# zhengchen1999/DOVE

Hardware: AMD Instinct MI355X
Metric: SR frames/s (33x720x1280 4x one-step, whole job) (higher is better)
Workload: dtype bf16; 1 GPU; synthetic 33x720x1280 HR clip (LR 180x320, 4x), one-step t=399, CogVideoX1.5-5B VAE + 42-layer DiT random-init, 1 clip per GPU (BASELINE configs[1]); weight_sums=True, vae_streams=2, variant=headline (bf16)

## Files before the change

### dove_amd/csrc/igemm.hip

```cpp
#include "igemm_args.h"


template <int BN, int BK>
struct FastCfg {
  static constexpr int BM = 128;
  static constexpr int CPR = BK / 8;
  static constexpr int CPR_LOG = (BK == 64) ? 3 : 2;
  static constexpr int RPG = 256 / CPR;
  static constexpr int NA = BM / RPG;
  static constexpr int B_SLOTS = BN * CPR;
  static constexpr int NB = (B_SLOTS + 255) / 256;
  static constexpr int A_BYTES = BM * BK * 2, B_BYTES = BN * BK * 2, STAGE = A_BYTES + B_BYTES;
  static constexpr int WN = (BN >= 128) ? 2 : 1, WM = 4 / WN;
  static constexpr int PT = (BM / WM) / 32, CT = (BN / WN) / 32;
  static constexpr int KK = BK / 16;
};

template <int BN, int BK>
__global__ __launch_bounds__(256) void igemm_fast_kernel(const IgemmArgs a) {
  using Cf = FastCfg<BN, BK>;
  constexpr int NA = Cf::NA, NB = Cf::NB, PT = Cf::PT, CT = Cf::CT, KK = Cf::KK, STAGE = Cf::STAGE, A_BYTES = Cf::A_BYTES;
  extern __shared__ __attribute__((aligned(16))) char smem[];
  const int tid = threadIdx.x, lane = tid & 63;
  const int wave = __builtin_amdgcn_readfirstlane(tid >> 6);
  __builtin_assume(wave >= 0 && wave < 4);
  const int wm = wave / Cf::WN, wn = wave % Cf::WN;

  unsigned rest = xcd_remap(blockIdx.x, gridDim.x);
  const int tn = rest % a.tiles_n; rest /= a.tiles_n;
  const int twi = rest % a.tiles_w; rest /= a.tiles_w;
  const int thi = rest % a.tiles_h;
  const int t = rest / a.tiles_h;
  const int n0 = tn * BN;
  const int TWm = (1 << a.tw_log2) - 1;
  const int oh0 = thi * (128 >> a.tw_log2), ow0 = twi << a.tw_log2;

  const int cs = tid & (Cf::CPR - 1);
  const int rsub = tid >> Cf::CPR_LOG;
  const int c = (BK == 64) ? (cs ^ ((rsub >> 1) & 7)) : (cs ^ ((rsub >> 2) & 3));
  int rowoff[NA];
  unsigned mask[NA];
#pragma unroll
  for (int j = 0; j < NA; ++j) {
    const int m = j * Cf::RPG + rsub;
    const int oh = oh0 + (m >> a.tw_log2), ow = ow0 + (m & TWm);
    const bool mv = (oh < a.H_out) && (ow < a.W_out);
    const int ih0 = oh * a.stride - a.pad_h, iw0 = ow * a.stride - a.pad_w;
    rowoff[j] = ((ih0 * a.W_in + iw0) * a.Cin + c * 8) * 2;
    unsigned mk = 0;
    for (int dh = 0; dh < a.kh; ++dh)
      for (int dw = 0; dw < a.kw; ++dw) {
        const bool ok = mv && ((unsigned)(ih0 + dh) < (unsigned)a.H_in) && ((unsigned)(iw0 + dw) < (unsigned)a.W_in);
        mk |= (ok ? 1u : 0u) << (dh * a.kw + dw);
      }
    mask[j] = mk;
  }
  int boff_g[NB];
#pragma unroll
  for (int j = 0; j < NB; ++j) boff_g[j] = ((j * Cf::RPG + rsub) * a.Cin + c * 8) * 2;

  const long long frame_elems = (long long)a.H_in * a.W_in * a.Cin;
  const unsigned frame_bytes = (unsigned)(frame_elems * 2);
  const unsigned wtap_bytes = (unsigned)((long long)BN * a.Cin * 2);
  const long long wtap_stride = (long long)a.Cout_pad * a.Cin;
  const int kc_per_tap = a.Cin / BK;
  const int nk = a.kt * a.kh * a.kw * kc_per_tap;

  auto frame_ptr = [&](int dt) -> const bf16_t* { return igemm_src_frame(a, t, dt, frame_elems); };
  int s_kc = 0, s_dw = 0, s_dh = 0, s_dt = 0;
  const bf16_t* s_fp = frame_ptr(0);
  const bf16_t* s_wp = a.w + (long long)n0 * a.Cin;
  int s_tapdelta = 0;
  unsigned s_tapbit = 1u;

// ... 23 lines not shown
          ++s_dt;
          if (s_dt < a.kt) s_fp = frame_ptr(s_dt);
        }
      }
      s_tapdelta = ((s_dh * a.W_in + s_dw) * a.Cin) * 2;
      s_tapbit = 1u << (s_dh * a.kw + s_dw);
    }
  };

  const int hi = lane >> 5, l31 = lane & 31;
  int aoff[PT][KK], boff[CT][KK];
#pragma unroll
  for (int kk = 0; kk < KK; ++kk) {
    const int chunk = kk * 2 + hi;
#pragma unroll
    for (int p = 0; p < PT; ++p) {
      const int row = wm * (Cf::BM / Cf::WM) + p * 32 + l31;
      const int sc = (BK == 64) ? (chunk ^ ((row >> 1) & 7)) : (chunk ^ ((row >> 2) & 3));
      aoff[p][kk] = row * (BK * 2) + sc * 16;
    }
#pragma unroll
    for (int i = 0; i < CT; ++i) {
      const int row = wn * (BN / Cf::WN) + i * 32 + l31;
      const int sc = (BK == 64) ? (chunk ^ ((row >> 1) & 7)) : (chunk ^ ((row >> 2) & 3));
      boff[i][kk] = row * (BK * 2) + sc * 16;
    }
  }

  f32x16 acc[CT][PT];
#pragma unroll
  for (int i = 0; i < CT; ++i)
#pragma unroll
    for (int p = 0; p < PT; ++p)
#pragma unroll
      for (int r = 0; r < 16; ++r) acc[i][p][r] = 0.f;

  auto compute = [&](auto bufc) {
    constexpr int BUF = decltype(bufc)::value;
#pragma unroll
    for (int kk = 0; kk < KK; ++kk) {
      bf16x8 xf[PT], wf[CT];
#pragma unroll
      for (int p = 0; p < PT; ++p) xf[p] = *(const bf16x8*)(smem + BUF * STAGE + aoff[p][kk]);
#pragma unroll
      for (int i = 0; i < CT; ++i) wf[i] = *(const bf16x8*)(smem + BUF * STAGE + A_BYTES + boff[i][kk]);
#pragma unroll
      for (int i = 0; i < CT; ++i)
#pragma unroll
        for (int p = 0; p < PT; ++p)
          acc[i][p] = __builtin_amdgcn_mfma_f32_32x32x16_bf16(wf[i], xf[p], acc[i][p], 0, 0, 0);
    }
  };

  using B0 = std::integral_constant<int, 0>;
  using B1 = std::integral_constant<int, 1>;
  stage(B0{});
  int it = 0;
  for (; it + 2 <= nk; it += 2) {
    asm volatile("s_waitcnt vmcnt(0)" ::: "memory");
    __syncthreads();
    stage(B1{});
    compute(B0{});
    asm volatile("s_waitcnt vmcnt(0)" ::: "memory");
    __syncthreads();
    if (it + 2 < nk) stage(B0{});
    compute(B1{});
  }
  if (nk & 1) {
    asm volatile("s_waitcnt vmcnt(0)" ::: "memory");
    __syncthreads();
    compute(B0{});
  }

#pragma unroll
  for (int p = 0; p < PT; ++p) {
    const int m = wm * (Cf::BM / Cf::WM) + p * 32 + l31;
    const int oh = oh0 + (m >> a.tw_log2), ow = ow0 + (m & TWm);
    if (!((oh < a.H_out) && (ow < a.W_out))) continue;
    const long long pix = ((long long)t * a.H_out + oh) * a.W_out + ow;
    const float* gate = a.gate ? (a.gate + (pix < a.gate_split ? 0 : a.Cout_pad)) : nullptr;
#pragma unroll
    for (int i = 0; i < CT; ++i) {
#pragma unroll
      for (int g = 0; g < 4; ++g) {
        const int cb = n0 + wn * (BN / Cf::WN) + i * 32 + 8 * g + 4 * hi;
        if (cb >= a.Cout_st) continue;
        float v[4];
#pragma unroll
        for (int e = 0; e < 4; ++e) v[e] = acc[i][p][g * 4 + e];
        if (a.bias) {
          const f32x4 b = *(const f32x4*)(a.bias + cb);
#pragma unroll
          for (int e = 0; e < 4; ++e) v[e] += b[e];
        }
        if (a.act == 1) {
#pragma unroll
          for (int e = 0; e < 4; ++e) v[e] = gelu_tanh_f(v[e]);
        }
        if (a.resid) {
          const uint2 rr = *(const uint2*)(a.resid + pix * a.ldr + cb);
          float r[4] = {__uint_as_float(rr.x << 16), __uint_as_float(rr.x & 0xffff0000u),
                        __uint_as_float(rr.y << 16), __uint_as_float(rr.y & 0xffff0000u)};
          if (gate) {
            const f32x4 gg = *(const f32x4*)(gate + cb);
#pragma unroll
            for (int e = 0; e < 4; ++e) v[e] = r[e] + gg[e] * v[e];
          } else {
#pragma unroll
            for (int e = 0; e < 4; ++e) v[e] += r[e];
          }
        }
        uint2 o;
        o.x = pack_bf2(v[0], v[1]);
        o.y = pack_bf2(v[2], v[3]);
        if (a.out_f32) *(f32x4*)((float*)a.out + pix * a.ldo + cb) = f32x4{v[0], v[1], v[2], v[3]};
        else *(uint2*)(a.out + pix * a.ldo + cb) = o;
      }
    }
  }
}


namespace halo8 {
constexpr int TH = 16, TW = 32, HWID = TW + 2, HHGT = TH + 2, HPIX = HWID * HHGT;
// ... 870 lines not shown
      for (int j = 0; j < 4; ++j)
        acc[j] = __builtin_amdgcn_fdot2_f32_bf16(__builtin_bit_cast(v2bf, wr[j][k]), __builtin_bit_cast(v2bf, xr[k]), acc[j], false);
    uint2 o;
    o.x = pack_bf2(acc[0], acc[1]);
    o.y = pack_bf2(acc[2], acc[3]);
    *(uint2*)(out + m * ldo + n0) = o;
  }
}

enum ConvKernel { K_IGEMM = 0, K_IGEMM_FAST, K_HALO4X, K_HALO4X_UP, K_GEMM8P, K_SMALLK, K_HALO4X_SUB };
static const char* const kKernelNames[] = {"igemm_kernel", "igemm_fast_kernel", "conv3x3_halo4x_kernel", "conv3x3_halo4x_kernel", "gemm8p_kernel",
                                           "smallk_kernel", "conv3x3_halo4x_kernel"};

static inline int desc_nb(const dove_conv_desc* d) { return d->nb > 1 ? d->nb : 1; }

static ConvKernel select_kernel(const dove_conv_desc* d) {
  const long long M = (long long)desc_nb(d) * d->t_out * d->h_out * d->w_out;
  const bool frame_fits = (long long)d->h_in * d->w_in * d->cin * 2 < (1ll << 31);
  const bool plain_gemm = d->kt == 1 && d->kh == 1 && d->kw == 1 && d->stride == 1 && d->up == 0 && d->tmode == 0 &&
                          d->t_in == d->t_out && d->h_in == d->h_out && d->w_in == d->w_out && d->cout_pad % 128 == 0 && M >= 4096 &&
                          (long long)512 * d->cin * 2 < (1ll << 31);
  const bool pointwise = d->kt == 1 && d->kh == 1 && d->kw == 1 && d->stride == 1 && d->up == 0 && d->tmode == 0 && d->t_in == d->t_out &&
                         d->h_in == d->h_out && d->w_in == d->w_out;
  if (pointwise && d->cin == 32 && d->act == 0 && !d->resid && !d->gate && d->cout_store >= 128) return K_SMALLK;
  if (plain_gemm) {
    if (d->cout_pad % 256 == 0 && d->cout_store % 256 == 0 && d->cin % 128 == 0 && d->cin >= 256 && (long long)256 * d->cin * 2 < (1ll << 31) &&
        d->ldo < (1 << 20) && d->ldr < (1 << 20) && (d->act == 0 || d->act == 1))
      return K_GEMM8P;
  }
  const bool conv3 = d->kh == 3 && d->kw == 3 && d->stride == 1 && d->pad_h == 1 && d->pad_w == 1 && d->act == 0 && !d->gate &&
                     d->cout_pad % 128 == 0 && frame_fits;
  if (conv3) {
    const bool same = d->up == 0 && d->tmode == 0 && d->h_out == d->h_in && d->w_out == d->w_in && d->w_out >= 16 && d->h_out >= 16;
    const bool ups = d->up == 1 && d->kt == 1 && d->h_out == 2 * d->h_in && d->w_out == 2 * d->w_in && d->h_out >= 16 && d->w_out >= 32;
    const bool h4 = d->cout_store % 128 == 0 && d->cin % 64 == 0 && d->ldo < (1 << 20) && (!d->resid || d->ldr < (1 << 20));
    if (same && h4) return K_HALO4X;
    if (ups && h4 && d->w_sub && d->h_in >= 16 && d->w_in >= 32) return K_HALO4X_SUB;
    if (ups && h4) return K_HALO4X_UP;
  }
  const int BN = (d->cout_pad % 128 == 0) ? 128 : ((d->cout_pad % 64 == 0) ? 64 : 32);
  const bool fits = frame_fits && (long long)BN * d->cin * 2 < (1ll << 31);
  return (d->up == 0 && fits) ? K_IGEMM_FAST : K_IGEMM;
}

static bool desc_size_ok(const dove_conv_desc* d, const char* who) {
  if (d && d->struct_size == sizeof(dove_conv_desc) && d->reserved == 0) return true;
  if (d) dove_set_error("%s: dove_conv_desc.struct_size is %u, this library (ABI %d) expects %zu - the caller's binding was written "
                        "against another include/dove_hip.h", who, d->struct_size, DOVE_ABI_VERSION, sizeof(dove_conv_desc));
  else dove_set_error("%s: null descriptor", who);
  return false;
}
extern "C" const char* dove_conv_kernel_name(const dove_conv_desc* d) { return desc_size_ok(d, "conv_kernel_name") ? kKernelNames[select_kernel(d)] : ""; }

template <int BN, int BK>
static int launch_igemm_fast(const IgemmArgs& a, unsigned grid, hipStream_t s) {
  constexpr int lds = 2 * (128 * BK * 2 + BN * BK * 2);
  static PerDeviceOnce attr_set;
  if (auto once_ = attr_set.guard()) (void)hipFuncSetAttribute((const void*)igemm_fast_kernel<BN, BK>, hipFuncAttributeMaxDynamicSharedMemorySize, lds);
  hipLaunchKernelGGL((igemm_fast_kernel<BN, BK>), dim3(grid), dim3(256), lds, s, a);
  DOVE_CHECK_LAUNCH("dove_conv_igemm_bf16");
  return DOVE_OK;
}

static int cu_count() {
  static std::atomic<int> cus[DOVE_MAX_DEVICES] = {};
  int dev = 0;
  (void)hipGetDevice(&dev);
  int n = (dev >= 0 && dev < DOVE_MAX_DEVICES) ? cus[dev].load(std::memory_order_relaxed) : 0;
  if (!n) {
    n = 256;
    (void)hipDeviceGetAttribute(&n, hipDeviceAttributeMultiprocessorCount, dev);
    if (dev >= 0 && dev < DOVE_MAX_DEVICES) cus[dev].store(n, std::memory_order_relaxed);
  }
  return n;
}

extern "C" long long dove_conv_gn_partial_rows(const dove_conv_desc* d) {
  if (!desc_size_ok(d, "conv_gn_partial_rows")) return 0;
  const ConvKernel k = select_kernel(d);
  if (k != K_HALO4X && k != K_HALO4X_UP && k != K_HALO4X_SUB) return 0;
  if (d->cout_store != 128 && d->cout_store != 256 && d->cout_store != 512) return 0;
  if (d->cout_store != d->cout_pad) return 0;
  if (k == K_HALO4X_SUB) {
    const long long th = (d->h_in + halo8::TH - 1) / halo8::TH, tw = (d->w_in + halo8::TW - 1) / halo8::TW;
    return (long long)desc_nb(d) * d->t_out * th * tw * 16;
  }
  const long long th = (d->h_out + halo8::TH - 1) / halo8::TH, tw = (d->w_out + halo8::TW - 1) / halo8::TW;
  return (long long)desc_nb(d) * d->t_out * th * tw * 4;
}

static bool halo4x_plan(const dove_conv_desc* d) {
  const int tiles_w = (d->w_out + halo8::TW - 1) / halo8::TW, tiles_h = (d->h_out + halo8::TH - 1) / halo8::TH;
  const int wrem = d->w_out % halo8::TW;
  if (wrem < 1 || wrem > halo8::TW / 2) return false;
  const int cus = cu_count();
  const long long per = (long long)desc_nb(d) * d->t_out * (d->cout_pad / 128);
  auto rounds = [&](long long tiles) { return (tiles * per + cus - 1) / cus; };
  return rounds((long long)tiles_h * (tiles_w - 1)) + rounds((d->h_out + 31) / 32) < rounds((long long)tiles_h * tiles_w);
}
extern "C" int dove_conv_partial_launches(const dove_conv_desc* d) {
  if (!desc_size_ok(d, "conv_partial_launches") || select_kernel(d) != K_HALO4X) return 0;
  return halo4x_plan(d) ? 1 : 0;
}

static int conv_dispatch(const dove_conv_desc* d, void* stream, ConvKernel kern);

static bool gemm_tail_split(const dove_conv_desc* d, long long* rows_main) {
  const long long M = (long long)d->t_out * d->h_out * d->w_out;
  if (d->t_out != 1 || d->h_out != 1 || desc_nb(d) > 1) return false;
  const int cus = cu_count(), tiles_n = d->cout_pad / 256;
  const long long row_tiles = (M + gemm4x::BM - 1) / gemm4x::BM, ntiles = row_tiles * tiles_n;
  if (ntiles <= cus || ntiles % cus == 0) return false;
  const long long main_rt = (ntiles / cus) * cus / tiles_n;
  if (main_rt < 1 || main_rt >= row_tiles) return false;
  const long long tail_rows = M - main_rt * gemm4x::BM;
  const long long tail_blocks = ((tail_rows + 127) / 128) * (d->cout_pad / 128);
  if (tail_blocks > 2ll * cus) return false;
  if ((long long)128 * d->cin * 2 >= (1ll << 31)) return false;
  *rows_main = main_rt * gemm4x::BM;
  return true;
}

extern "C" int dove_conv_igemm_bf16(const dove_conv_desc* d, void* stream) {
  if (!desc_size_ok(d, "conv_igemm")) return DOVE_EINVAL;
  DOVE_CHECK_ARG(d->x && d->w && d->out, "conv_igemm: null pointer");
  DOVE_CHECK_ARG(d->cin % 32 == 0 && d->cin > 0, "conv_igemm: Cin (%d) must be a positive multiple of 32 (pad on pack)", d->cin);
  DOVE_CHECK_ARG(d->cout_pad % 32 == 0 && d->cout_pad > 0, "conv_igemm: Cout_pad (%d) must be a multiple of 32", d->cout_pad);
  DOVE_CHECK_ARG(d->cout_store % 4 == 0 && d->cout_store <= d->cout_pad && d->cout_store > 0, "conv_igemm: bad cout_store %d", d->cout_store);
  DOVE_CHECK_ARG(d->ldo % 4 == 0 && d->ldo >= d->cout_store, "conv_igemm: ldo (%lld) must be a multiple of 4 and >= cout_store", d->ldo);
  DOVE_CHECK_ARG(!d->resid || (d->ldr % 4 == 0 && d->ldr >= d->cout_store), "conv_igemm: bad ldr %lld", d->ldr);
  DOVE_CHECK_ARG(!d->gate || d->resid, "conv_igemm: gate needs resid");
  DOVE_CHECK_ARG(d->kt >= 1 && d->kt <= 3 && d->kh >= 1 && d->kw >= 1, "conv_igemm: bad kernel size");
  DOVE_CHECK_ARG(d->stride == 1 || d->stride == 2, "conv_igemm: stride must be 1 or 2");
  DOVE_CHECK_ARG(d->up == 0 || d->up == 1, "conv_igemm: up must be 0/1");
  DOVE_CHECK_ARG(d->kt == 1 || (d->tmode == 0 && d->t_in == d->t_out), "conv_igemm: causal temporal taps need t_in == t_out and tmode 0");
  DOVE_CHECK_ARG(d->t_out > 0 && d->h_out > 0 && d->w_out > 0 && d->t_in > 0 && d->h_in > 0 && d->w_in > 0, "conv_igemm: empty tensor");
  DOVE_CHECK_ARG(d->nb >= 0 && d->nb <= 4096 && (long long)desc_nb(d) * d->t_out < (1 << 20), "conv_igemm: bad instance count nb = %d", d->nb);
  DOVE_CHECK_ARG(d->cache_stride == 0 || (d->cache && d->cache_stride >= (long long)(d->kt - 1) * d->h_in * d->w_in * d->cin),
                 "conv_igemm: cache_stride (%lld) is smaller than one instance's cache", d->cache_stride);
  DOVE_CHECK_ARG(desc_nb(d) == 1 || !d->gate, "conv_igemm: nb > 1 is not combined with gate");
  DOVE_CHECK_ARG(d->reserved2 == 0 && d->tdup >= 0 && d->tdup <= 2, "conv_igemm: bad tdup %d", d->tdup);
  DOVE_CHECK_ARG(!d->tdup || (d->kt == 3 && d->w_pair), "conv_igemm: tdup declares frame pairs of a kt == 3 conv and needs w_pair");
  DOVE_CHECK_ARG(!d->tdup || d->cache || d->w_first, "conv_igemm: tdup without a conv cache needs w_first too (frames whose three taps read one frame)");
  DOVE_CHECK_ARG(d->tdup != 2 || !d->cache, "conv_igemm: tdup == 2 (first frame single) is the head of a clip: no conv cache");
  DOVE_CHECK_ARG(!d->gn_partial || dove_conv_gn_partial_rows(d) > 0,
                 "conv_igemm: gn_partial requested but this call does not dispatch to a kernel that fuses the statistics");
  const ConvKernel kern0 = select_kernel(d);
  DOVE_CHECK_ARG(!d->out_f32 || (kern0 == K_IGEMM_FAST && !d->resid && d->act == 0),
                 "conv_igemm: out_f32 is only implemented for plain convs that dispatch to igemm_fast_kernel");
  long long rows_main = 0;
  if (kern0 == K_GEMM8P && gemm_tail_split(d, &rows_main)) {
    dove_conv_desc m = *d, t = *d;
    m.w_in = m.w_out = (int)rows_main;
    const long long tail = (long long)d->w_out - rows_main;
    t.w_in = t.w_out = (int)tail;
    t.x = (const char*)d->x + rows_main * d->cin * 2;
    t.out = (char*)d->out + rows_main * d->ldo * 2;
    if (d->resid) t.resid = (const char*)d->resid + rows_main * d->ldr * 2;
    t.gate_split = d->gate_split > rows_main ? d->gate_split - rows_main : 0;
    const int rc = conv_dispatch(&m, stream, K_GEMM8P);
    return rc ? rc : conv_dispatch(&t, stream, K_IGEMM_FAST);
  }
  return conv_dispatch(d, stream, kern0);
}

static int conv_dispatch(const dove_conv_desc* d, void* stream, ConvKernel kern) {
  const bf16_t* zp = zero_page();
  DOVE_CHECK_ARG(zp, "conv_igemm: could not allocate the zero page");
  IgemmArgs a;
  a.x = (const bf16_t*)d->x; a.cache = (const bf16_t*)d->cache; a.w = (const bf16_t*)d->w;
  a.bias = d->bias; a.resid = (const bf16_t*)d->resid; a.gate = d->gate; a.out = (bf16_t*)d->out; a.zero = zp;
  const int nb = desc_nb(d);
  a.T_out = nb * d->t_out; a.H_out = d->h_out; a.W_out = d->w_out;
  a.T_in = nb * d->t_in; a.H_in = d->h_in; a.W_in = d->w_in;
  a.seg_out = d->t_out; a.seg_in = d->t_in;
  a.cache_bs = d->cache_stride ? d->cache_stride : (long long)(d->kt - 1) * d->h_in * d->w_in * d->cin;
  a.Cin = d->cin; a.Cout_pad = d->cout_pad; a.Cout_st = d->cout_store;
  a.kt = d->kt; a.kh = d->kh; a.kw = d->kw; a.stride = d->stride; a.pad_h = d->pad_h; a.pad_w = d->pad_w;
  a.up = d->up; a.tmode = d->tmode; a.act = d->act; a.ldo = d->ldo; a.ldr = d->ldr; a.gate_split = d->gate_split;
  a.gn_partial = nullptr; a.cpg_log = 0;
  a.w_first = nullptr;
  a.w_pair = nullptr; a.tdup = 0;
  a.sub = 0;
  a.out_f32 = d->out_f32;
  a.nt_out = 0;
  a.reserved = 0;
  hipStream_t s = (hipStream_t)stream;
  const long long M = (long long)nb * d->t_out * d->h_out * d->w_out;
  switch (kern) {
    case K_GEMM8P: {
      a.tiles_n = d->cout_pad / 256;
      a.nt_out = (long long)M * d->ldo * 2 > (256ll << 20);
      const long long nt = ((M + gemm4x::BM - 1) / gemm4x::BM) * a.tiles_n;
      DOVE_CHECK_ARG(nt > 0 && nt < (1ll << 31), "conv_igemm: grid too large");
      DOVE_CHECK_ARG(!(d->gate && d->act), "conv_igemm: gate with activation is not a path of the reference");
      const int cus = cu_count();
      const unsigned grid4 = nt > cus ? (unsigned)cus : (unsigned)nt;
      static PerDeviceOnce attr8;
      if (auto once_ = attr8.guard()) {
        (void)hipFuncSetAttribute((const void*)gemm8p_kernel<false, false>, hipFuncAttributeMaxDynamicSharedMemorySize, gemm8p::LDS_BYTES);
        (void)hipFuncSetAttribute((const void*)gemm8p_kernel<true, false>, hipFuncAttributeMaxDynamicSharedMemorySize, gemm8p::LDS_BYTES);
        (void)hipFuncSetAttribute((const void*)gemm8p_kernel<false, true>, hipFuncAttributeMaxDynamicSharedMemorySize, gemm8p::LDS_BYTES);
      }
      if (d->gate) hipLaunchKernelGGL((gemm8p_kernel<false, true>), dim3(grid4), dim3(512), gemm8p::LDS_BYTES, s, a, M);
      else if (d->act == 1) hipLaunchKernelGGL((gemm8p_kernel<true, false>), dim3(grid4), dim3(512), gemm8p::LDS_BYTES, s, a, M);
      else hipLaunchKernelGGL((gemm8p_kernel<false, false>), dim3(grid4), dim3(512), gemm8p::LDS_BYTES, s, a, M);
      DOVE_CHECK_LAUNCH("dove_conv_igemm_bf16(gemm8p)");
      return DOVE_OK;
    }
    case K_SMALLK: {
      dim3 grid((unsigned)((M + 4 * smallk::ROWS - 1) / (4 * smallk::ROWS)), (unsigned)((d->cout_store + 255) / 256));
      hipLaunchKernelGGL(smallk_kernel, grid, dim3(256), 0, s, a.x, a.w, a.bias, a.out, M, d->cout_store, d->ldo);
      DOVE_CHECK_LAUNCH("dove_conv_igemm_bf16(smallk)");
      return DOVE_OK;
    }
    case K_HALO4X_SUB: {
      a.gn_partial = d->gn_partial;
      a.cpg_log = d->cout_store == 128 ? 2 : (d->cout_store == 256 ? 3 : 4);
      a.sub = 1;
// ... 4 lines not shown
      a.tiles_n = 4 * (d->cout_pad / 128);
      a.nty = a.tiles_h; a.ntx = a.tiles_w; a.h_lim = d->h_out; a.w_lim = d->w_out;
      const long long g4 = (long long)a.T_out * a.tiles_h * a.tiles_w * a.tiles_n;
      DOVE_CHECK_ARG(g4 > 0 && g4 < (1ll << 31), "conv_igemm: grid too large");
      static PerDeviceOnce attrs;
      if (auto once_ = attrs.guard()) (void)hipFuncSetAttribute((const void*)(conv3x3_halo4x_kernel<false, true>), hipFuncAttributeMaxDynamicSharedMemorySize, Halo4xCfg::LDS_BYTES);
      const int cus = cu_count();
      const unsigned grid = g4 > cus ? (unsigned)cus : (unsigned)g4;
      hipLaunchKernelGGL((conv3x3_halo4x_kernel<false, true>), dim3(grid), dim3(256), Halo4xCfg::LDS_BYTES, s, a);
      DOVE_CHECK_LAUNCH("dove_conv_igemm_bf16(halo4x sub-pixel)");
      return DOVE_OK;
    }
    case K_HALO4X:
    case K_HALO4X_UP: {
      a.gn_partial = d->gn_partial;
      a.w_first = (kern == K_HALO4X && d->kt == 3 && !d->cache) ? (const bf16_t*)d->w_first : nullptr;
      if (kern == K_HALO4X && d->kt == 3 && d->tdup) { a.tdup = d->tdup; a.w_pair = (const bf16_t*)d->w_pair; }
      a.cpg_log = d->cout_store == 128 ? 2 : (d->cout_store == 256 ? 3 : 4);
      a.tiles_w = (d->w_out + halo8::TW - 1) / halo8::TW;
      a.tiles_h = (d->h_out + halo8::TH - 1) / halo8::TH;
      a.tiles_n = d->cout_pad / 128;
      a.ty0 = a.tx0 = 0; a.nty = a.tiles_h; a.ntx = a.tiles_w; a.h_lim = d->h_out; a.w_lim = d->w_out;
      const long long g4 = (long long)a.T_out * a.tiles_h * a.tiles_w * a.tiles_n;
      DOVE_CHECK_ARG(g4 > 0 && g4 < (1ll << 31), "conv_igemm: grid too large");
      static PerDeviceOnce attr4;
      if (auto once_ = attr4.guard()) {
        (void)hipFuncSetAttribute((const void*)(conv3x3_halo4x_kernel<false>), hipFuncAttributeMaxDynamicSharedMemorySize, Halo4xCfg::LDS_BYTES);
        (void)hipFuncSetAttribute((const void*)(conv3x3_halo4x_kernel<false, false, 1>), hipFuncAttributeMaxDynamicSharedMemorySize, H4Geo<1>::LDS_BYTES);
        (void)hipFuncSetAttribute((const void*)(conv3x3_halo4x_kernel<true>), hipFuncAttributeMaxDynamicSharedMemorySize, Halo4xCfg::LDS_BYTES);
      }
      const int cus = cu_count();
      const unsigned grid = g4 > cus ? (unsigned)cus : (unsigned)g4;
      if (kern == K_HALO4X_UP) hipLaunchKernelGGL((conv3x3_halo4x_kernel<true>), dim3(grid), dim3(256), Halo4xCfg::LDS_BYTES, s, a);
      else {
        const bool wpart = halo4x_plan(d);
        const int wm = wpart ? (a.tiles_w - 1) * halo8::TW : d->w_out, cols_main = wpart ? a.tiles_w - 1 : a.tiles_w;
        auto launch = [&](int part, int nty, int tx0, int ntx, int w_lim) {
          if (nty <= 0 || ntx <= 0) return;
          IgemmArgs b = a;
          b.ty0 = 0; b.nty = nty; b.tx0 = tx0; b.ntx = ntx; b.h_lim = d->h_out; b.w_lim = w_lim;
          const long long g = (long long)b.T_out * nty * ntx * b.tiles_n;
          const unsigned gr = g > cus ? (unsigned)cus : (unsigned)g;
          if (part == 0) hipLaunchKernelGGL((conv3x3_halo4x_kernel<false, false, 0>), dim3(gr), dim3(256), H4Geo<0>::LDS_BYTES, s, b);
          else hipLaunchKernelGGL((conv3x3_halo4x_kernel<false, false, 1>), dim3(gr), dim3(256), H4Geo<1>::LDS_BYTES, s, b);
        };
        launch(0, a.tiles_h, 0, cols_main, wm);
        if (wpart) launch(1, (d->h_out + 31) / 32, cols_main, 1, d->w_out);
      }
      DOVE_CHECK_LAUNCH("dove_conv_igemm_bf16(halo4x)");
      return DOVE_OK;
    }
    default: break;
  }
  int twl = 7;
  if (d->h_out > 1) {
    twl = 4;
    if (d->w_out <= 8) twl = 3;
    if (d->w_out <= 4) twl = 2;
  }
  a.tw_log2 = twl;
  const int TW = 1 << twl, TH = 128 >> twl;
  a.tiles_w = (d->w_out + TW - 1) / TW;
  a.tiles_h = (d->h_out + TH - 1) / TH;
  const int BN = (d->cout_pad % 128 == 0) ? 128 : ((d->cout_pad % 64 == 0) ? 64 : 32);
  a.tiles_n = d->cout_pad / BN;
  const long long grid = (long long)a.T_out * a.tiles_h * a.tiles_w * a.tiles_n;
  DOVE_CHECK_ARG(grid > 0 && grid < (1ll << 31), "conv_igemm: grid too large");
  const bool fast = kern == K_IGEMM_FAST;
  const bool bk64 = (d->cin % 64 == 0);
  if (!fast) return launch_igemm_legacy(a, (unsigned)grid, BN, bk64, s);
  if (BN == 128) return bk64 ? launch_igemm_fast<128, 64>(a, (unsigned)grid, s) : launch_igemm_fast<128, 32>(a, (unsigned)grid, s);
  if (BN == 64) return bk64 ? launch_igemm_fast<64, 64>(a, (unsigned)grid, s) : launch_igemm_fast<64, 32>(a, (unsigned)grid, s);
  return bk64 ? launch_igemm_fast<32, 64>(a, (unsigned)grid, s) : launch_igemm_fast<32, 32>(a, (unsigned)grid, s);
}
```

### dove_amd/lib.py

```python
from __future__ import annotations

import ctypes as C
import os

import torch

_HERE = os.path.dirname(os.path.abspath(__file__))
LIB_PATH = os.path.join(_HERE, "libdove_hip.so")
_lib = None

F32, BF16, U8 = 0, 1, 2
METRIC_PSNR, METRIC_SSIM, METRIC_RGB_TO_Y = 1, 2, 4
COLORFIX_WAVELET, COLORFIX_ADAIN, COLORFIX_CLAMP = 1, 2, 1
YUV_444, YUV_422, YUV_420, YUV_MONO = 0, 1, 2, 3
YUV_SITING_LEFT, YUV_SITING_CENTRE = 0, 1
VIDEO_RGB_U8, VIDEO_YUV = 0, 1
RESIZE_BILINEAR, RESIZE_BICUBIC, RESIZE_AREA = 0, 1, 2
ACT_NONE, ACT_RELU, ACT_SIGMOID, ACT_TANH = 0, 1, 2, 3


class ConvDesc(C.Structure):
    _fields_ = [
        ("struct_size", C.c_uint), ("reserved", C.c_uint),
        ("x", C.c_void_p), ("cache", C.c_void_p), ("w", C.c_void_p), ("bias", C.c_void_p),
# ... 144 lines not shown
    "dove_shard_frames": [_VP, _I, _I, C.POINTER(C.c_int), C.POINTER(C.c_int)],
    "dove_conv_out_gather_cl": [_VP, _LL, _I, _I, _I, _I, _VP, _VP, _I, _VP],
    "dove_tile_gather_bf16": [_VP, _I, _I, _I, _I, _I, _I, _I, _I, C.POINTER(C.c_int), C.POINTER(C.c_int), _I, _VP, _VP],
    "dove_linear_mxfp8": [_VP, _VP, _VP, _VP, _VP, _VP, _VP, _VP, _LL, _I, _I, _LL, _LL, _LL, _I, _VP],
    "dove_fr_metrics": [C.POINTER(ImageView), C.POINTER(ImageView), _I, _I, _I, _I, _I, _VP, C.c_size_t, _VP, _VP],
    "dove_color_fix": [C.POINTER(ImageView), _F, _F, C.POINTER(ImageView), _F, _F, _I, _I, _I, _I, _I, C.POINTER(ImageView), _VP,
                       C.c_size_t, _VP],
    "dove_rgb_to_yuv_u8": [C.POINTER(ImageView), _I, _I, _I, C.POINTER(YuvFormat), _VP, _VP],
    "dove_yuv_to_rgb_u8": [_VP, _I, _I, _I, C.POINTER(YuvFormat), _VP, _VP],
    "dove_plan_padding": [_I, _I, _I, _PI, _PI, _PI],
    "dove_plan_output_size": [_I, _I, _I, _PI, _PI],
    "dove_plan_temporal_chunks": [_I, _I, _I, _PI, _I],
    "dove_plan_spatial_tiles": [_I, _I, _I, _I, _I, _I, _PI, _I],
    "dove_plan_valid_region": [_PI, _I, _I, _I, _I, _I, _I, _PI, _PI],
    "dove_plan_pieces": [_I, _I, _I, _I, _I, _I, _I, _I, _I, _PI, _PI, _PI, _I],
    "dove_plan_check_coverage": [_PI, _I, _I, _I, _I],
    "dove_chunk_planner_create": [_I, _I, C.POINTER(_VP)],
    "dove_chunk_planner_next": [_VP, _LL, _I, _PLL, _PLL, _PI],
    "dove_philox_u32": [_VP, _LL, _ULL, _ULL, _ULL, _VP],
    "dove_randn": [_VP, _I, _LL, _ULL, _ULL, _ULL, _VP],
    "dove_blur2d_f32": [_VP, _I, _I, _I, _VP, _I, _I, _VP, _VP],
    "dove_resize_f32": [_VP, _I, _I, _I, _I, _I, _I, _VP, _VP],
    "dove_add_gaussian_noise_f32": [_VP, _I, _I, _I, C.POINTER(C.c_float), _I, _ULL, _ULL, _LL, _VP, _VP],
    "dove_add_poisson_noise_f32": [_VP, _I, _I, _I, C.POINTER(C.c_float), _I, _ULL, _ULL, _LL, _VP, C.c_size_t, _VP, _VP],
    "dove_jpeg_roundtrip": [_VP, _I, _I, _I, _PI, _VP, C.c_size_t, _VP, _VP],
    "dove_stitch": [_VP, _I, _I, _I, _PI, _VP, _I, _I, _I, _I, _I, _I, _VP],
    "dove_video_open": [_VP, C.POINTER(VideoParams), C.POINTER(_VP)],
    "dove_video_info": [_VP, C.POINTER(C.c_size_t), C.POINTER(C.c_size_t), _PI, _PI, _PI],
    "dove_video_push": [_VP, _VP, _I, _VP],
    "dove_video_end_of_input": [_VP],
    "dove_video_need": [_VP, _PLL, _PI],
    "dove_video_step": [_VP, _VP, C.c_size_t, _PI, _PI, _VP],
    "dove_conv2d_f32": [C.POINTER(Conv2dF32Args), _VP],
    "dove_instance_norm_f32": [_VP, _I, _I, _I, _I, _VP, _I, _F, _VP, C.c_size_t, _VP, _VP],
    "dove_corr_volume_f32": [_VP, _VP, _I, _I, _I, _I, _F, _VP, _VP],
    "dove_avgpool2_f32": [_VP, _LL, _I, _I, _VP, _VP],
    "dove_corr_lookup_f32": [_VP, _VP, _VP, _VP, _VP, _LL, _I, _I, _I, _I, _VP, _VP],
    "dove_gru_gate_f32": [_VP, _LL, _VP, _LL, _I, _I, _LL, _VP, _VP],
    "dove_gru_update_f32": [_VP, _LL, _VP, _LL, _VP, _LL, _I, _LL, _VP],
    "dove_add_f32": [_VP, _LL, _VP, _LL, _VP, _LL, _I, _LL, _I, _VP],
    "dove_convex_upsample_f32": [_VP, _LL, _VP, _I, _I, _I, _VP, _VP],
    "dove_flow_warp_error": [_VP, _VP, _I, _VP, _VP, _I, _I, _I, _VP, C.c_size_t, _VP, _VP, _VP, _VP],
    "dove_convnet_conv_f32": [C.POINTER(ConvnetConvF32Args), _VP],
    "dove_percep_prep_f32": [C.POINTER(ImageView), _I, _I, _I, _I, _F, _F, C.POINTER(C.c_float), C.POINTER(C.c_float), _VP, _VP],
    "dove_maxpool_f32": [_VP, _LL, _I, _I, _I, _I, _I, _I, _VP, _LL, _VP],
    "dove_l2pool_f32": [_VP, _LL, _I, _I, _I, _I, _VP, _LL, _VP],
    "dove_lpips_layer": [_VP, _VP, _LL, _VP, _I, _I, _I, _I, _VP, C.c_size_t, _VP, _VP],
    "dove_dists_layer": [_VP, _VP, _LL, _VP, _VP, _I, _I, _I, _I, _VP, C.c_size_t, _VP, _VP],
}
PLAIN = {"dove_last_error": (C.c_char_p, []), "dove_abi_version": (C.c_int, []), "dove_comm_destroy": (None, [C.c_void_p]),
         "dove_conv_gn_partial_rows": (C.c_longlong, [C.POINTER(ConvDesc)]),
         "dove_conv_kernel_name": (C.c_char_p, [C.POINTER(ConvDesc)]),
         "dove_conv_partial_launches": (C.c_int, [C.POINTER(ConvDesc)]),
         "dove_attention_head_paths": (C.c_int, [C.POINTER(C.c_float), _I, C.POINTER(C.c_int)]),
         "dove_attention_path_name": (C.c_char_p, [_I]),
         "dove_device_info": (C.c_int, [_I, C.c_char_p, _I, C.POINTER(C.c_int), C.POINTER(C.c_longlong)]),
         "dove_destroy": (None, [_VP]),
         "dove_vae_decode_num_frames": (C.c_int, [_VP, _I]),
         "dove_get_option": (C.c_longlong, [_VP, _I]),
         "dove_comm_useful_ranks": (C.c_int, [_VP, _I, _I]),
         "dove_workspace_bytes": (C.c_size_t, [_VP, _I, _I, _I]),
         "dove_workspace_high_water": (C.c_size_t, [_VP]),
         "dove_fr_metrics_workspace_bytes": (C.c_size_t, [_I, _I, _I]),
         "dove_color_fix_workspace_bytes": (C.c_size_t, [_I, _I, _I, _I]),
         "dove_yuv_frame_bytes": (C.c_size_t, [_I, _I, _I]),
         "dove_poisson_noise_workspace_bytes": (C.c_size_t, [_I]),
         "dove_jpeg_roundtrip_workspace_bytes": (C.c_size_t, [_I, _I, _I]),
         "dove_chunk_planner_need": (C.c_longlong, [_VP]),
         "dove_chunk_planner_destroy": (None, [_VP]),
         "dove_video_workspace_bytes": (C.c_size_t, [_VP, C.POINTER(VideoParams)]),
         "dove_video_close": (None, [_VP]),
         "dove_instance_norm_f32_workspace_bytes": (C.c_size_t, [_I, _I, _I, _I]),
         "dove_flow_warp_error_workspace_bytes": (C.c_size_t, [_I, _I, _I]),
         "dove_convnet_conv_f32_kernel_name": (C.c_char_p, [C.POINTER(ConvnetConvF32Args)]),
         "dove_lpips_layer_workspace_bytes": (C.c_size_t, [_I, _I, _I]),
         "dove_dists_layer_workspace_bytes": (C.c_size_t, [_I, _I, _I, _I])}


def kernel_source_sha256() -> str:
    import glob
    import hashlib
    h = hashlib.sha256()
    files = sorted(glob.glob(os.path.join(_HERE, "csrc", "*.hip")) + glob.glob(os.path.join(_HERE, "csrc", "*.h")))
    files.append(os.path.join(os.path.dirname(_HERE), "include", "dove_hip.h"))
    for fn in files:
        h.update(os.path.basename(fn).encode() + b"\0")
        with open(fn, "rb") as f:
            h.update(f.read())
        h.update(b"\0")
    return h.hexdigest()


def load():
    global _lib
    if _lib is not None:
        return _lib
    if not os.path.exists(LIB_PATH):
        raise RuntimeError(f"{LIB_PATH} not found: build it with `python -c 'import __graft_entry__ as g; g.build()'` "
                           "(dove_amd has no CPU fallback)")
    lib = C.CDLL(LIB_PATH)
    for name, argt in SIGNATURES.items():
        fn = getattr(lib, name)
        fn.argtypes = argt
        fn.restype = C.c_int
    for name, (res, argt) in PLAIN.items():
        fn = getattr(lib, name)
# ... 41 lines not shown
```

### dove_amd/ops.py

```python
from __future__ import annotations

import ctypes as C
import math
from dataclasses import dataclass

import torch

from . import lib as L


def _ru(x: int, m: int) -> int:
    return (x + m - 1) // m * m


@dataclass
class PackedConv:
    w: torch.Tensor
    bias: torch.Tensor | None
    kt: int
    kh: int
    kw: int
    cin: int
    cin_pad: int
    cout: int
# ... 24 lines not shown
        bp[:cout] = bias.detach().to(device=device, dtype=torch.float32)
    wp = wp.contiguous()
    w_first = None
    if kt == 3:
        t = wp.float().view(3, kh * kw, cout_pad, cin_pad)
        s01 = t[0] + t[1]
        w_first = torch.stack([s01, s01 + t[2]]).to(torch.bfloat16).contiguous()
    w_pair = None
    if kt == 3 and pair:
        t = wp.float().view(3, kh * kw, cout_pad, cin_pad)
        w_pair = torch.stack([t[0] + t[1], t[1] + t[2]]).to(torch.bfloat16).contiguous()
    w_sub = None
    if kt == 1 and kh == 3 and kw == 3 and sub:
        t = wp.float().view(3, 3, cout_pad, cin_pad)
        w_sub = torch.zeros(4, 4, cout_pad, cin_pad, dtype=torch.float32, device=device)
        for py in range(2):
            for px in range(2):
                for dh in range(3):
                    for dw in range(3):
                        a, b = (py + dh + 1) // 2 - py, (px + dw + 1) // 2 - px
                        w_sub[2 * py + px, 2 * a + b] += t[dh, dw]
        w_sub = w_sub.to(torch.bfloat16).contiguous()
    return PackedConv(wp, bp, kt, kh, kw, cin, cin_pad, cout, cout_pad, w_first, w_sub, w_pair)


def temporal_split(tl: int, tdup: int, cached: bool, first_sums: bool = True):
    plain = [("w0", tl - 2), ("w1", tl - 1), ("w2", tl)]
    if tdup == 0:
        if cached or not first_sums or tl > 1:
            return plain
        return [("w012", 0)] if tl == 0 else [("w01", 0), ("w2", 1)]
    if tdup == 1:
        if not cached and tl < 2:
            return [("w012", tl)]
        return [("w0", tl - 2), ("w12", tl)] if tl & 1 else [("w01", tl - 1), ("w2", tl)]
    if tl == 0:
        return [("w012", 0)]
    return [("w01", tl - 1), ("w2", tl)] if tl & 1 else [("w0", tl - 2), ("w12", tl)]


def temporal_groups(tl: int, tdup: int, cached: bool) -> int:
    return len(temporal_split(tl, tdup, cached))


_profiler = None


def set_profiler(records: list | None):
    global _profiler
    _profiler = records


def conv_kernel_name(x_shape, pc: PackedConv, *, stride=1, pad=(None, None), up=0, tmode=0, t_out=None, hw_out=None, act=0, gated=False,
                     resid=False, nb=1, partial=False):
    T, H, W, Cx = x_shape
    d = L.ConvDesc()
    d.nb = nb
    ph = (pc.kh - 1) // 2 if pad[0] is None else pad[0]
    pw = (pc.kw - 1) // 2 if pad[1] is None else pad[1]
    t_out = T if t_out is None else t_out
    if hw_out is None:
        hw_out = (H << up, W << up) if stride == 1 else ((H + 1 - pc.kh) // stride + 1, (W + 1 - pc.kw) // stride + 1)
    d.t_in, d.h_in, d.w_in, d.cin = T, H, W, Cx
    d.t_out, d.h_out, d.w_out = t_out, hw_out[0], hw_out[1]
    d.cout_pad, d.cout_store = pc.cout_pad, pc.cout_store
    d.kt, d.kh, d.kw, d.stride, d.pad_h, d.pad_w = pc.kt, pc.kh, pc.kw, stride, ph, pw
    d.up, d.tmode, d.act = up, tmode, act
    d.ldo = pc.cout_store
    d.ldr = pc.cout_store if resid else 0
    d.resid = 1 if (resid or gated) else None
    d.w_sub = 1 if (up == 1 and pc.kt == 1 and pc.kh == 3 and pc.kw == 3) else None
    d.gate = 1 if gated else None
    if partial:
        return int(L.load().dove_conv_partial_launches(C.byref(d)))
    return L.load().dove_conv_kernel_name(C.byref(d)).decode()


def conv(x: torch.Tensor, pc: PackedConv, *, cache: torch.Tensor | None = None, stride: int = 1, pad=(None, None),
         up: int = 0, tmode: int = 0, t_out: int | None = None, hw_out=None, resid: torch.Tensor | None = None,
         gate: torch.Tensor | None = None, gate_split: int = 0, act: int = 0, ldo: int | None = None,
         out: torch.Tensor | None = None,
         gn_eps: float | None = None, out_f32: bool = False, nb: int = 1, tdup: int = 0, weight_sums: bool = True) -> torch.Tensor:
    L.require_cuda(x, resid, gate, out)
    assert x.dtype == torch.bfloat16 and x.dim() == 4, (x.dtype, x.shape)
    T, H, W, Cx = x.shape
    assert T % nb == 0, (T, nb)
    T //= nb
    if Cx != pc.cin_pad:
        raise RuntimeError(f"conv: input has {Cx} channels, packed weight expects {pc.cin_pad}")
    ph = (pc.kh - 1) // 2 if pad[0] is None else pad[0]
    pw = (pc.kw - 1) // 2 if pad[1] is None else pad[1]
    if t_out is None:
        t_out = T
    if hw_out is None:
        hw_out = (H << up, W << up) if stride == 1 else ((H + 1 - pc.kh) // stride + 1, (W + 1 - pc.kw) // stride + 1)
    if ldo is None:
        ldo = pc.cout_store
    odt = torch.float32 if out_f32 else torch.bfloat16
    if out is None:
        out = torch.empty(nb * t_out, hw_out[0], hw_out[1], ldo, dtype=odt, device=x.device)
    else:
        assert out.shape == (nb * t_out, hw_out[0], hw_out[1], ldo) and out.dtype == odt
    cache_stride = 0
    if cache is not None:
        if nb > 1:
            assert cache.shape == (nb, pc.kt - 1, H, W, Cx) and cache.dtype == torch.bfloat16 and cache.is_cuda, (cache.shape, x.shape)
            assert cache[0].is_contiguous() and cache.device == x.device
            cache_stride = cache.stride(0)
        else:
            L.require_cuda(cache)
            assert cache.shape == (pc.kt - 1, H, W, Cx) and cache.dtype == torch.bfloat16, (cache.shape, x.shape)
    d = L.ConvDesc()
    d.nb, d.cache_stride = nb, cache_stride
    if cache is None and pc.w_first is not None and weight_sums:
        d.w_first = pc.w_first.data_ptr()
    if up == 1 and pc.w_sub is not None and weight_sums:
        d.w_sub = pc.w_sub.data_ptr()
    if tdup and weight_sums and pc.w_pair is not None and pc.kt == 3 and not (tdup == 2 and cache is not None):
        d.tdup, d.w_pair = tdup, pc.w_pair.data_ptr()
    d.x, d.cache, d.w = x.data_ptr(), (cache.data_ptr() if cache is not None else None), pc.w.data_ptr()
    d.bias = pc.bias.data_ptr() if pc.bias is not None else None
    d.resid = resid.data_ptr() if resid is not None else None
    d.gate = gate.data_ptr() if gate is not None else None
    d.out = out.data_ptr()
    d.t_in, d.h_in, d.w_in, d.cin = T, H, W, Cx
    d.t_out, d.h_out, d.w_out = t_out, hw_out[0], hw_out[1]
    d.cout_pad, d.cout_store = pc.cout_pad, pc.cout_store
# ... 866 lines not shown
```

### include/dove_hip.h

```cpp
#ifndef DOVE_HIP_H
#define DOVE_HIP_H

#include <stddef.h>

#ifdef __cplusplus
extern "C" {
#endif

#define DOVE_ABI_VERSION 15

#define DOVE_F32 0
#define DOVE_BF16 1

const char* dove_last_error(void);
int dove_abi_version(void);
int dove_device_info(int dev, char* name, int name_len, int* cu_count, long long* total_mem);

typedef struct dove_conv_desc {
  unsigned int struct_size;
  unsigned int reserved;
  const void* x;
  const void* cache;
  const void* w;
  const float* bias;
  const void* resid;
  const float* gate;
  void* out;
  int t_in, h_in, w_in, cin;
  int t_out, h_out, w_out, cout_pad, cout_store;
  int kt, kh, kw, stride, pad_h, pad_w, up, tmode, act;
  long long ldo, ldr, gate_split;
  float* gn_partial;
  int out_f32;
  int nb;
  long long cache_stride;
  const void* w_first;
  const void* w_sub;
  const void* w_pair;
  int tdup;
  int reserved2;
} dove_conv_desc;
int dove_conv_igemm_bf16(const dove_conv_desc* d, void* stream);
const char* dove_conv_kernel_name(const dove_conv_desc* d);
int dove_conv_partial_launches(const dove_conv_desc* d);
long long dove_conv_gn_partial_rows(const dove_conv_desc* d);
int dove_groupnorm_finalize_partials(const float* partial, long long rows, double count, float eps, void* ws, float* stats,
                                     void* stream);

int dove_groupnorm_stats_bf16(const void* x, long long npix, long long frame_pix, int C, float eps, void* partial_ws, int ws_blocks,
                              float* stats, void* stream);
int dove_groupnorm_sums_bf16(const void* x, long long npix, long long frame_pix, int C, void* partial_ws, int ws_blocks, double* sums,
                             void* stream);
int dove_groupnorm_finalize_sums(const double* sums, double count, float eps, float* stats, void* stream);
int dove_groupnorm_sums_from_partials(const float* partial, long long rows, void* ws, double* sums, void* stream);
int dove_groupnorm_apply_bf16(const void* x, void* y, int T, int H, int W, int C, const float* stats,
                              const float* gamma, const float* beta, int silu, const void* yb, int hz, int wz,
                              int sshift, const int* tmap, void* stream);

int dove_groupnorm_stats_nb_bf16(const void* x, int nb, long long npix, long long frame_pix, int C, float eps, void* partial_ws,
                                 int ws_blocks, float* stats, void* stream);
int dove_groupnorm_finalize_partials_nb(const float* partial, long long rows, int nb, double count, float eps, void* ws, size_t ws_bytes,
                                        float* stats, void* stream);
int dove_groupnorm_apply_nb_bf16(const void* x, void* y, int nb, int T, int H, int W, int C, const float* stats, const float* gamma,
                                 const float* beta, int silu, const void* yb, int Tz, int hz, int wz, int sshift, const int* tmap,
                                 void* stream);
int dove_avgpool_time_nb_bf16(const void* x, int nb, int T, long long frame_elems, void* y, void* stream);

int dove_layernorm_modulate_bf16(const void* x, void* y, long long rows, int D, float eps, const float* gamma,
                                 const float* beta, const float* mod, long long split, void* stream);

int dove_qkv_post_bf16(const void* qkv, long long N, long long Npad, int heads, int head_dim, int text_len,
                       const float* gq, const float* bq, const float* gk, const float* bk, const float* cosT,
                       const float* sinT, float qscale, float eps, void* Qh, void* Kh, void* Vt, int v_order, float* norm2, void* stream);
int dove_vt_quad_swap_bf16(void* Vt, long long rows, long long Npad, void* stream);
int dove_ulysses_place_bf16(const void* rq, const void* rk, const void* rv, const long long* counts, int world, int hloc, long long N,
                            long long Npad, void* Qh, void* Kh, void* Vt, float* norm2_out, void* stream);

int dove_attention_fwd_bf16(const void* Qh, const void* Kh, const void* Vt, void* O, long long N, long long Npad,
                            int heads, int head_dim, long long ldo, float* norm2, void* stream);
int dove_attention_head_paths(const float* norm2_host, int heads, int* path);
const char* dove_attention_path_name(int path);

int dove_cl_from_ncthw(const void* x, int dtype, int C, long long npix, int Cp, float scale, float shift, void* y,
                       void* stream);
int dove_ncthw_from_cl(const void* x, long long ld, int C, long long npix, float scale, float shift, float lo,
                       float hi, void* y, int dtype, void* stream);
int dove_cl_im2col3x3_from_ncthw(const void* x, int dtype, int C, int T, int H, int W, int Cp, float scale, float shift, void* y,
                                 void* stream);
int dove_conv_out_gather(const float* p, long long ldp, int T, int H, int W, int C, const float* bias, float scale, float shift, float lo,
                         float hi, void* y, int dtype, void* stream);
int dove_avgpool_time_bf16(const void* x, int T, long long frame_elems, void* y, void* stream);
int dove_posterior_sample(const void* moments, long long ld, int latent_channels, long long npix, const void* noise,
                          int noise_dtype, void* out, int out_dtype, void* stream);
int dove_axpby(const void* x, const void* y, void* out, int dtype, long long n, float a, float b, void* stream);
int dove_patchify(const void* x, int dtype, int T, int C, int H, int W, int pt, int p, void* tokens, long long ld,
                  void* stream);
int dove_unpatchify(const void* tokens, long long ld, int T, int C, int H, int W, int pt, int p, void* y, int dtype,
// ... 249 lines not shown
```

Baseline: 35.86 frames/s.

## Add multi-stage LDS ring pipeline to igemm_fast with occupancy-aware stage count

Replaces the double-buffered main loop of the fast implicit-GEMM conv kernel with an S-stage ring buffer that keeps up to S-1 tile loads in flight. It waits on a partial vmcnt rather than draining all loads, and uses one barrier per stage. A host-side plan picks the stage count: 4 stages when the grid fits in one wave of CUs, 3 for BN128/BK32, otherwise 2. The GEMM tail-split heuristic is also reworked to use the plan's residency. Deeper rings use more LDS, which can reduce occupancy, and only small grids get the deepest pipeline.

New measurement: 35.81 frames/s, median of 2. No clear change (-0.1%).

```diff
diff --git a/dove_amd/csrc/igemm.hip b/dove_amd/csrc/igemm.hip
--- a/dove_amd/csrc/igemm.hip
+++ b/dove_amd/csrc/igemm.hip
@@ -1,5 +1,7 @@
 #include "igemm_args.h"
 
+
+constexpr int kCuLdsBytes = 160 << 10;
 
 template <int BN, int BK>
 struct FastCfg {
@@ -16,10 +18,27 @@
   static constexpr int KK = BK / 16;
 };
 
-template <int BN, int BK>
+template <int N>
+__device__ __forceinline__ void fast_wait_vm() {
+  static_assert(N >= 0 && N <= 63, "vmcnt has 6 bits");
+  asm volatile("s_waitcnt vmcnt(%0)" ::"n"(N) : "memory");
+}
+template <int NLD, int A>
+__device__ __forceinline__ void fast_ring_wait(int ahead) {
+  if constexpr (A == 0) fast_wait_vm<0>();
+  else {
+    if (ahead >= A) fast_wait_vm<NLD * A>();
+    else fast_ring_wait<NLD, A - 1>(ahead);
+  }
+}
+template <int... J, class F>
+__device__ __forceinline__ void fast_static_for(std::integer_sequence<int, J...>, F&& f) { (f(std::integral_constant<int, J>{}), ...); }
+
+template <int BN, int BK, int S>
 __global__ __launch_bounds__(256) void igemm_fast_kernel(const IgemmArgs a) {
   using Cf = FastCfg<BN, BK>;
   constexpr int NA = Cf::NA, NB = Cf::NB, PT = Cf::PT, CT = Cf::CT, KK = Cf::KK, STAGE = Cf::STAGE, A_BYTES = Cf::A_BYTES;
+  static_assert(S >= 2 && (NA + NB) * (S - 1) <= 63, "the ring's outstanding LDS-DMAs must fit vmcnt");
   extern __shared__ __attribute__((aligned(16))) char smem[];
   const int tid = threadIdx.x, lane = tid & 63;
   const int wave = __builtin_amdgcn_readfirstlane(tid >> 6);
@@ -149,24 +168,28 @@
     }
   };
 
-  using B0 = std::integral_constant<int, 0>;
-  using B1 = std::integral_constant<int, 1>;
-  stage(B0{});
-  int it = 0;
-  for (; it + 2 <= nk; it += 2) {
-    asm volatile("s_waitcnt vmcnt(0)" ::: "memory");
-    __syncthreads();
-    stage(B1{});
-    compute(B0{});
-    asm volatile("s_waitcnt vmcnt(0)" ::: "memory");
-    __syncthreads();
-    if (it + 2 < nk) stage(B0{});
-    compute(B1{});
-  }
-  if (nk & 1) {
-    asm volatile("s_waitcnt vmcnt(0)" ::: "memory");
-    __syncthreads();
-    compute(B0{});
+  constexpr int B_REM = Cf::B_SLOTS % 256;
+  auto ring_wait = [&](int ahead) {
+    if constexpr (B_REM == 0) fast_ring_wait<NA + NB, S - 2>(ahead);
+    else {
+      if (wave * 64 < B_REM) fast_ring_wait<NA + NB, S - 2>(ahead);
+      else fast_ring_wait<NA + NB - 1, S - 2>(ahead);
+    }
+  };
+  fast_static_for(std::make_integer_sequence<int, S - 1>{}, [&](auto jc) {
+    if (decltype(jc)::value < nk) stage(jc);
+  });
+  for (int it = 0; it < nk; it += S) {
+    fast_static_for(std::make_integer_sequence<int, S>{}, [&](auto jc) {
+      constexpr int J = decltype(jc)::value;
+      const int s = it + J;
+      if (s < nk) {
+        ring_wait(nk - 1 - s);
+        __builtin_amdgcn_s_barrier();
+        if (s + S - 1 < nk) stage(std::integral_constant<int, (J + S - 1) % S>{});
+        compute(jc);
+      }
+    });
   }
 
 #pragma unroll
@@ -1143,15 +1166,20 @@
 }
 extern "C" const char* dove_conv_kernel_name(const dove_conv_desc* d) { return desc_size_ok(d, "conv_kernel_name") ? kKernelNames[select_kernel(d)] : ""; }
 
-template <int BN, int BK>
+template <int BN, int BK, int S>
 static int launch_igemm_fast(const IgemmArgs& a, unsigned grid, hipStream_t s) {
-  constexpr int lds = 2 * (128 * BK * 2 + BN * BK * 2);
+  constexpr int lds = S * FastCfg<BN, BK>::STAGE;
+  static_assert(lds <= kCuLdsBytes, "a ring must fit one CU's LDS");
   static PerDeviceOnce attr_set;
-  if (auto once_ = attr_set.guard()) (void)hipFuncSetAttribute((const void*)igemm_fast_kernel<BN, BK>, hipFuncAttributeMaxDynamicSharedMemorySize, lds);
-  hipLaunchKernelGGL((igemm_fast_kernel<BN, BK>), dim3(grid), dim3(256), lds, s, a);
+  if (auto once_ = attr_set.guard()) (void)hipFuncSetAttribute((const void*)igemm_fast_kernel<BN, BK, S>, hipFuncAttributeMaxDynamicSharedMemorySize, lds);
+  hipLaunchKernelGGL((igemm_fast_kernel<BN, BK, S>), dim3(grid), dim3(256), lds, s, a);
   DOVE_CHECK_LAUNCH("dove_conv_igemm_bf16");
   return DOVE_OK;
 }
+
+#define DOVE_FAST_INSTANCES(X) \
+  X(128, 64, 2); X(128, 64, 4); X(128, 32, 2); X(128, 32, 3); X(128, 32, 4); X(64, 64, 2); X(64, 64, 4); X(64, 32, 2); X(64, 32, 4); \
+  X(32, 64, 2); X(32, 64, 4); X(32, 32, 2); X(32, 32, 4);
 
 static int cu_count() {
   static std::atomic<int> cus[DOVE_MAX_DEVICES] = {};
@@ -1166,6 +1194,27 @@
   return n;
 }
 
+struct FastPlan {
+  int bn, bk, stages;
+  int tw_log2, tiles_w, tiles_h;
+  long long grid;
+  int lds() const { return stages * (128 + bn) * bk * 2; }
+  int resident() const { return kCuLdsBytes / lds(); }
+};
+static FastPlan fast_plan(const dove_conv_desc* d) {
+  FastPlan p;
+  p.tw_log2 = 7;
+  if (d->h_out > 1) p.tw_log2 = d->w_out <= 4 ? 2 : (d->w_out <= 8 ? 3 : 4);
+  const int TW = 1 << p.tw_log2, TH = 128 >> p.tw_log2;
+  p.tiles_w = (d->w_out + TW - 1) / TW;
+  p.tiles_h = (d->h_out + TH - 1) / TH;
+  p.bn = (d->cout_pad % 128 == 0) ? 128 : ((d->cout_pad % 64 == 0) ? 64 : 32);
+  p.grid = (long long)desc_nb(d) * d->t_out * p.tiles_h * p.tiles_w * (d->cout_pad / p.bn);
+  p.bk = (d->cin % 64 == 0) ? 64 : 32;
+  p.stages = p.grid <= cu_count() ? 4 : ((p.bn == 128 && p.bk == 32) ? 3 : 2);
+  return p;
+}
+
 extern "C" long long dove_conv_gn_partial_rows(const dove_conv_desc* d) {
   if (!desc_size_ok(d, "conv_gn_partial_rows")) return 0;
   const ConvKernel k = select_kernel(d);
@@ -1194,22 +1243,41 @@
   return halo4x_plan(d) ? 1 : 0;
 }
 
-static int conv_dispatch(const dove_conv_desc* d, void* stream, ConvKernel kern);
-
-static bool gemm_tail_split(const dove_conv_desc* d, long long* rows_main) {
+static int conv_dispatch(const dove_conv_desc* d, void* stream, ConvKernel kern, const FastPlan* plan = nullptr);
+
+static bool gemm_tail_split(const dove_conv_desc* d, long long* rows_main, dove_conv_desc* tail_desc, FastPlan* tail_plan) {
   const long long M = (long long)d->t_out * d->h_out * d->w_out;
   if (d->t_out != 1 || d->h_out != 1 || desc_nb(d) > 1) return false;
   const int cus = cu_count(), tiles_n = d->cout_pad / 256;
   const long long row_tiles = (M + gemm4x::BM - 1) / gemm4x::BM, ntiles = row_tiles * tiles_n;
   if (ntiles <= cus || ntiles % cus == 0) return false;
+  if (2 * (ntiles % cus) >= cus) return false;
   const long long main_rt = (ntiles / cus) * cus / tiles_n;
   if (main_rt < 1 || main_rt >= row_tiles) return false;
-  const long long tail_rows = M - main_rt * gemm4x::BM;
-  const long long tail_blocks = ((tail_rows + 127) / 128) * (d->cout_pad / 128);
-  if (tail_blocks > 2ll * cus) return false;
   if ((long long)128 * d->cin * 2 >= (1ll << 31)) return false;
-  *rows_main = main_rt * gemm4x::BM;
+  const long long rows = main_rt * gemm4x::BM, tail = M - rows;
+  dove_conv_desc t = *d;
+  t.w_in = t.w_out = (int)tail;
+  t.x = (const char*)d->x + rows * d->cin * 2;
+  t.out = (char*)d->out + rows * d->ldo * 2;
+  if (d->resid) t.resid = (const char*)d->resid + rows * d->ldr * 2;
+  t.gate_split = d->gate_split > rows ? d->gate_split - rows : 0;
+  const FastPlan p = fast_plan(&t);
+  if (p.grid > (long long)p.resident() * cus) return false;
+  *rows_main = rows;
+  *tail_desc = t;
+  *tail_plan = p;
   return true;
+}
+
+extern "C" int dove_conv_igemm_stages(const dove_conv_desc* d) {
+  if (!desc_size_ok(d, "conv_igemm_stages")) return 0;
+  const ConvKernel k = select_kernel(d);
+  long long rows_main = 0;
+  dove_conv_desc t;
+  FastPlan p;
+  if (k == K_GEMM8P) return gemm_tail_split(d, &rows_main, &t, &p) ? p.stages : 0;
+  return k == K_IGEMM_FAST ? fast_plan(d).stages : 0;
 }
 
 extern "C" int dove_conv_igemm_bf16(const dove_conv_desc* d, void* stream) {
@@ -1240,22 +1308,18 @@
   DOVE_CHECK_ARG(!d->out_f32 || (kern0 == K_IGEMM_FAST && !d->resid && d->act == 0),
                  "conv_igemm: out_f32 is only implemented for plain convs that dispatch to igemm_fast_kernel");
   long long rows_main = 0;
-  if (kern0 == K_GEMM8P && gemm_tail_split(d, &rows_main)) {
-    dove_conv_desc m = *d, t = *d;
+  dove_conv_desc t;
+  FastPlan tp;
+  if (kern0 == K_GEMM8P && gemm_tail_split(d, &rows_main, &t, &tp)) {
+    dove_conv_desc m = *d;
     m.w_in = m.w_out = (int)rows_main;
-    const long long tail = (long long)d->w_out - rows_main;
-    t.w_in = t.w_out = (int)tail;
-    t.x = (const char*)d->x + rows_main * d->cin * 2;
-    t.out = (char*)d->out + rows_main * d->ldo * 2;
-    if (d->resid) t.resid = (const char*)d->resid + rows_main * d->ldr * 2;
-    t.gate_split = d->gate_split > rows_main ? d->gate_split - rows_main : 0;
     const int rc = conv_dispatch(&m, stream, K_GEMM8P);
-    return rc ? rc : conv_dispatch(&t, stream, K_IGEMM_FAST);
+    return rc ? rc : conv_dispatch(&t, stream, K_IGEMM_FAST, &tp);
   }
   return conv_dispatch(d, stream, kern0);
 }
 
-static int conv_dispatch(const dove_conv_desc* d, void* stream, ConvKernel kern) {
+static int conv_dispatch(const dove_conv_desc* d, void* stream, ConvKernel kern, const FastPlan* plan) {
   const bf16_t* zp = zero_page();
   DOVE_CHECK_ARG(zp, "conv_igemm: could not allocate the zero page");
   IgemmArgs a;
@@ -1366,24 +1430,18 @@
     }
     default: break;
   }
-  int twl = 7;
-  if (d->h_out > 1) {
-    twl = 4;
-    if (d->w_out <= 8) twl = 3;
-    if (d->w_out <= 4) twl = 2;
-  }
-  a.tw_log2 = twl;
-  const int TW = 1 << twl, TH = 128 >> twl;
-  a.tiles_w = (d->w_out + TW - 1) / TW;
-  a.tiles_h = (d->h_out + TH - 1) / TH;
-  const int BN = (d->cout_pad % 128 == 0) ? 128 : ((d->cout_pad % 64 == 0) ? 64 : 32);
-  a.tiles_n = d->cout_pad / BN;
-  const long long grid = (long long)a.T_out * a.tiles_h * a.tiles_w * a.tiles_n;
-  DOVE_CHECK_ARG(grid > 0 && grid < (1ll << 31), "conv_igemm: grid too large");
-  const bool fast = kern == K_IGEMM_FAST;
-  const bool bk64 = (d->cin % 64 == 0);
-  if (!fast) return launch_igemm_legacy(a, (unsigned)grid, BN, bk64, s);
-  if (BN == 128) return bk64 ? launch_igemm_fast<128, 64>(a, (unsigned)grid, s) : launch_igemm_fast<128, 32>(a, (unsigned)grid, s);
-  if (BN == 64) return bk64 ? launch_igemm_fast<64, 64>(a, (unsigned)grid, s) : launch_igemm_fast<64, 32>(a, (unsigned)grid, s);
-  return bk64 ? launch_igemm_fast<32, 64>(a, (unsigned)grid, s) : launch_igemm_fast<32, 32>(a, (unsigned)grid, s);
-}
+  const FastPlan p = plan ? *plan : fast_plan(d);
+  a.tw_log2 = p.tw_log2;
+  a.tiles_w = p.tiles_w;
+  a.tiles_h = p.tiles_h;
+  a.tiles_n = d->cout_pad / p.bn;
+  DOVE_CHECK_ARG(p.grid > 0 && p.grid < (1ll << 31), "conv_igemm: grid too large");
+  const unsigned grid = (unsigned)p.grid;
+  if (kern != K_IGEMM_FAST) return launch_igemm_legacy(a, grid, p.bn, d->cin % 64 == 0, s);
+#define DOVE_FAST_CASE(BN_, BK_, S_) \
+  if (p.bn == BN_ && p.bk == BK_ && p.stages == S_) return launch_igemm_fast<BN_, BK_, S_>(a, grid, s)
+  DOVE_FAST_INSTANCES(DOVE_FAST_CASE)
+#undef DOVE_FAST_CASE
+  dove_set_error("conv_igemm: no igemm_fast instantiation <%d, %d, %d>", p.bn, p.bk, p.stages);
+  return DOVE_EINVAL;
+}
diff --git a/dove_amd/lib.py b/dove_amd/lib.py
--- a/dove_amd/lib.py
+++ b/dove_amd/lib.py
@@ -220,6 +220,7 @@
          "dove_conv_gn_partial_rows": (C.c_longlong, [C.POINTER(ConvDesc)]),
          "dove_conv_kernel_name": (C.c_char_p, [C.POINTER(ConvDesc)]),
          "dove_conv_partial_launches": (C.c_int, [C.POINTER(ConvDesc)]),
+         "dove_conv_igemm_stages": (C.c_int, [C.POINTER(ConvDesc)]),
          "dove_attention_head_paths": (C.c_int, [C.POINTER(C.c_float), _I, C.POINTER(C.c_int)]),
          "dove_attention_path_name": (C.c_char_p, [_I]),
          "dove_device_info": (C.c_int, [_I, C.c_char_p, _I, C.POINTER(C.c_int), C.POINTER(C.c_longlong)]),
diff --git a/dove_amd/ops.py b/dove_amd/ops.py
--- a/dove_amd/ops.py
+++ b/dove_amd/ops.py
@@ -100,7 +100,7 @@
 
 
 def conv_kernel_name(x_shape, pc: PackedConv, *, stride=1, pad=(None, None), up=0, tmode=0, t_out=None, hw_out=None, act=0, gated=False,
-                     resid=False, nb=1, partial=False):
+                     resid=False, nb=1, partial=False, stages=False):
     T, H, W, Cx = x_shape
     d = L.ConvDesc()
     d.nb = nb
@@ -121,6 +121,8 @@
     d.gate = 1 if gated else None
     if partial:
         return int(L.load().dove_conv_partial_launches(C.byref(d)))
+    if stages:
+        return int(L.load().dove_conv_igemm_stages(C.byref(d)))
     return L.load().dove_conv_kernel_name(C.byref(d)).decode()
 
 
diff --git a/include/dove_hip.h b/include/dove_hip.h
--- a/include/dove_hip.h
+++ b/include/dove_hip.h
@@ -43,6 +43,7 @@
 int dove_conv_igemm_bf16(const dove_conv_desc* d, void* stream);
 const char* dove_conv_kernel_name(const dove_conv_desc* d);
 int dove_conv_partial_launches(const dove_conv_desc* d);
+int dove_conv_igemm_stages(const dove_conv_desc* d);
 long long dove_conv_gn_partial_rows(const dove_conv_desc* d);
 int dove_groupnorm_finalize_partials(const float* partial, long long rows, double count, float eps, void* ws, float* stats,
                                      void* stream);
```
